# rogeliorjr/DyCON_Paper_Replication

Hardware: AMD Instinct MI355X
Metric: train volumes/sec (96^3 patch) (higher is better)
Workload: dtype bf16

## Files before the change

### dycon_paper_replication_amd/_lib.py

```python
from __future__ import annotations

import ctypes as C
import os

_HERE = os.path.dirname(os.path.abspath(__file__))
LIB_PATH = os.environ.get("DYCON_LIB", os.path.join(_HERE, "libdycon_hip.so"))

F32, BF16 = 0, 1
CONV_1X1, CONV_K3, CONV_K2S2 = 0, 1, 2

P, I, L, F, Z, U64 = C.c_void_p, C.c_int, C.c_longlong, C.c_float, C.c_size_t, C.c_uint64

SIGNATURES = {
    "dycon_version": (I, []),
    "dycon_last_error": (C.c_char_p, []),
    "dycon_bfrag_bytes": (Z, [I, I, I, I]),
    "dycon_pack_bfrag": (I, [P, P, I, I, I, I, I, L, L, L, L, I, P]),
    "dycon_pack_batch": (I, [P, I, I, P]),
    "dycon_pack_tcn": (I, [P, P, I, I, I, I, L, L, L, L, I, P]),
    "dycon_conv_gemm_workspace": (Z, [I, I, I, I, I, I, I, I, I]),
    "dycon_conv_gemm_plan": (I, [I, I, I, I, I, I, I, I, I, I, I, P]),
    "dycon_conv_kernel_name": (C.c_char_p, [I]),
    "dycon_conv_region_name": (C.c_char_p, [P]),
    "dycon_conv_gemm": (I, [P, P, P, P, I, I, I, I, I, I, I, I, I, I, I, P, Z, P]),
    "dycon_conv_gemm_splits": (I, [I, I, I, I, I, I, I, I, I]),
    "dycon_conv_gemm_ex": (I, [P, P, P, P, I, I, I, I, I, I, I, I, I, I, I, P, Z, I, P]),
    "dycon_conv_direct": (I, [P, I, P, P, P, I, I, I, I, I, I, I, I, I, P]),
    "dycon_conv_wgrad_workspace": (Z, [I, I, I, I, I, I, I]),
    "dycon_conv_wgrad_name": (C.c_char_p, [I, I, I, I, I, I, I, I, I]),
    "dycon_conv_wgrad": (I, [P, I, P, I, P, P, I, I, I, I, I, I, I, L, L, L, P, Z, P]),
    "dycon_colsum_workspace": (Z, [L, I]),
    "dycon_colsum": (I, [P, I, P, L, I, P, Z, P]),
    "dycon_norm_workspace": (Z, [I, L, I]),
    "dycon_norm_stats": (I, [P, I, I, L, I, I, F, P, P, P, F, P, Z, P]),
    "dycon_norm_fwd": (I, [P, P, I, I, L, I, I, F, P, P, P, I, P, P, P, P, F, P, Z, P]),
    "dycon_norm_fwd_is_fused": (I, [I, L, I, I]),
    "dycon_norm_fwd_slab": (I, [P, I, P, P, P, I, I, L, I, I, F, P, P, P, I, P, P, P]),
    "dycon_norm_apply": (I, [P, P, I, I, L, I, I, P, P, P, I, P, P, P]),
    "dycon_norm_bwd": (I, [P, I, P, P, I, I, L, I, I, P, P, P, I, P, P, P, P, Z, P]),
    "dycon_norm_bwd_ex": (I, [P, I, P, P, I, I, L, I, I, P, P, P, I, P, P, P, I, P, Z, P]),
    "dycon_norm_sum_dparams": (I, [P, I, I, P, P, P]),
    "dycon_norm_head_workspace": (Z, [I, L]),
    "dycon_norm_head_fwd": (I, [P, I, I, L, I, P, P, P, I, P, P, P, P, P]),
    "dycon_norm_head_bwd": (I, [P, P, P, I, I, L, I, P, P, P, I, P, P, P, P, P, Z, P]),
    "dycon_norm_head_dparams": (I, [P, I, L, P, P, P]),
    "dycon_norm_headc_workspace": (Z, [I, L, I]),
    "dycon_norm_headc_fwd": (I, [P, I, I, L, I, I, P, P, P, I, P, P, P, P, P]),
# ... 106 lines not shown
    "dycon_sample_colsum": (I, [P, I, P, I, L, I, F, I, P]),
    "dycon_sample_bcast": (I, [P, P, P, I, I, L, I, F, P]),
    "dycon_small_gemm": (I, [P, L, L, P, L, L, P, L, I, I, I, I, P]),
    "dycon_copy_segments": (I, [P, P, P, I, P]),
    "dycon_assemble_batch": (I, [P, P, P, I, I, I, I, P, P, I, P]),
    "dycon_sw_gather": (I, [P, I, I, I, P, I, I, I, I, I, I, P, P]),
    "dycon_sw_accumulate_ens": (I, [P, P, P, P, I, I, I, I, I, I, P, P, P, I, I, I, P]),
    "dycon_volume_stats_workspace": (Z, [I, L]),
    "dycon_volume_stats": (I, [P, I, L, P, P, P, Z, P]),
    "dycon_normalize_apply": (I, [P, I, L, P, P, P]),
    "dycon_zoom_workspace": (Z, [I, I, I, I]),
    "dycon_zoom": (I, [P, I, I, I, I, I, I, I, I, I, P, I, F, P, I, P, Z, P]),
    "dycon_kernel_timing": (I, [I]),
    "dycon_kernel_timing_count": (L, []),
    "dycon_kernel_timing_fetch": (I, [L, L, P, P, P]),
    "dycon_kernel_timing_name": (C.c_char_p, [I]),
}


class ConvPlan(C.Structure):
    _fields_ = [("family", I), ("splits", I), ("chunks", I), ("weights", I), ("workspace", Z)]


CONV_NONE, CONV_C1, CONV_P16, CONV_P32, CONV_LDS, CONV_HALO, CONV_TILE, CONV_GEMM = range(8)
CONV_W_FRAG, CONV_W_CHUNK16 = 0, 1


class View(C.Structure):
    _fields_ = [("p", P), ("sn", L), ("sc", L), ("sv", L)]


class DyconLibraryError(RuntimeError):
    pass


_lib = None


def load():
    global _lib
    if _lib is not None:
        return _lib
    if not os.path.exists(LIB_PATH):
        raise DyconLibraryError(
            f"{LIB_PATH} not found: the HIP extension is not built.  Run "
            "`python -c 'import __graft_entry__ as g; g.build()'` from the repo root.  "
            "There is no CPU/PyTorch fallback for the DyCON hot path.")
# ... 95 lines not shown
```

### dycon_paper_replication_amd/csrc/conv.hip

```cpp
#include <stdlib.h>

#include "common.h"

typedef float f32x4 __attribute__((ext_vector_type(4)));
typedef __bf16 bf16x8 __attribute__((ext_vector_type(8)));

template <typename T> struct Frag;
template <> struct Frag<float> { static constexpr int G = 4, KC = 16; };
template <> struct Frag<bf16> { static constexpr int G = 8, KC = 32; };

__device__ __forceinline__ void mma(f32x4& acc, const Vec16<float>& a, const Vec16<float>& b) {
    acc = __builtin_amdgcn_mfma_f32_16x16x4f32(a.v.x, b.v.x, acc, 0, 0, 0);
    acc = __builtin_amdgcn_mfma_f32_16x16x4f32(a.v.y, b.v.y, acc, 0, 0, 0);
    acc = __builtin_amdgcn_mfma_f32_16x16x4f32(a.v.z, b.v.z, acc, 0, 0, 0);
    acc = __builtin_amdgcn_mfma_f32_16x16x4f32(a.v.w, b.v.w, acc, 0, 0, 0);
}
__device__ __forceinline__ void mma(f32x4& acc, const Vec16<bf16>& a, const Vec16<bf16>& b) {
    acc = __builtin_amdgcn_mfma_f32_16x16x32_bf16(__builtin_bit_cast(bf16x8, a.v), __builtin_bit_cast(bf16x8, b.v),
                                                  acc, 0, 0, 0);
}

template <int MODE> __device__ __forceinline__ int n_taps() { return MODE == DYCON_CONV_K3 ? 27 : MODE == DYCON_CONV_K2S2 ? 8 : 1; }

template <int MODE>
__device__ __forceinline__ bool src_voxel(int t, int z, int y, int x, int Di, int Hi, int Wi, int& zi, int& yi, int& xi) {
    if (MODE == DYCON_CONV_K3) {
        const int dz = t / 9, dy = (t / 3) % 3, dx = t % 3;
        zi = z + dz - 1; yi = y + dy - 1; xi = x + dx - 1;
        return (unsigned)zi < (unsigned)Di && (unsigned)yi < (unsigned)Hi && (unsigned)xi < (unsigned)Wi;
    } else if (MODE == DYCON_CONV_K2S2) {
        zi = 2 * z + (t >> 2); yi = 2 * y + ((t >> 1) & 1); xi = 2 * x + (t & 1);
        return true;
    } else {
        zi = z; yi = y; xi = x;
        return true;
    }
}

template <typename T>
__global__ void pack_bfrag_kernel(const float* __restrict__ w, T* __restrict__ out, int Tn, int Cin, int N, int N0,
                                  long long s_t, long long s_c, long long s_n1, long long s_n0, int flip, int NT,
                                  long long total) {
    constexpr int G = Frag<T>::G, KC = Frag<T>::KC;
    for (long long i = (long long)blockIdx.x * blockDim.x + threadIdx.x; i < total; i += (long long)gridDim.x * blockDim.x) {
        const int e = (int)(i % G);
        long long q = i / G;
        const int lane = (int)(q % 64);
        q /= 64;
        const int nt = (int)(q % NT);
        const int kc = (int)(q / NT);
        const int k = kc * KC + G * (lane >> 4) + e;
        const int n = nt * 16 + (lane & 15);
        float v = 0.f;
        if (k < Tn * Cin && n < N) {
            int t = k / Cin;
            const int c = k - t * Cin;
            if (flip) t = Tn - 1 - t;
            v = w[t * s_t + c * s_c + (long long)(n / N0) * s_n1 + (long long)(n % N0) * s_n0];
        }
        stf(out + i, v);
// ... 2548 lines not shown
    if (!(B > 0 && Di > 0 && Hi > 0 && Wi > 0 && Cin > 0 && N > 0 && Cout > 0)) return {"conv_gemm: bad shape", 0};
    if (mode < 0 || mode > 2) return {"conv_gemm: bad mode %d", mode};
    if (!conv_first_layer(dtype, mode, scatter, Di, Hi, Wi, Cin, Cout) && Cin % (dtype == DYCON_BF16 ? 8 : 4) != 0)
        return {"conv_gemm: Cin=%d not a multiple of the fragment width", Cin};
    if (N % 16 != 0) return {"conv_gemm: N=%d not a multiple of 16 (use dycon_conv_direct)", N};
    if (scatter && !(mode == DYCON_CONV_1X1 && N == 8 * Cout)) return {"conv_gemm: scatter needs mode 1x1 and N == 8*Cout", 0};
    if (!scatter && N != Cout) return {"conv_gemm: N must equal Cout without scatter", 0};
    if (mode == DYCON_CONV_K2S2 && (Di % 2 || Hi % 2 || Wi % 2)) return {"conv_gemm: k2s2 needs even dims", 0};
    return {nullptr, 0};
}
struct ConvPlan {
    int family = DYCON_CONV_NONE;
    int variant = 0;
    int ck = 0, ntb = 0;
    bool wide = false;
    int tz = 0, ty = 0, tx = 0, nTiles = 0;
    dim3 grid;
    long long M = 0;
    SplitK sk{1, 0};
    int splits = 1;
    size_t ws_bytes = 0;
    int chunks = 0;
    int weights = DYCON_CONV_W_FRAG;
};
static ConvPlan conv_fwd_plan(int dtype, int mode, int scatter, int accumulate, int B, int Di, int Hi, int Wi, int Cin, int N, int Cout) {
    ConvPlan p;
    if (B <= 0 || Di <= 0 || Hi <= 0 || Wi <= 0 || Cin <= 0 || N <= 0 || Cout <= 0 || mode < 0 || mode > 2) return p;
    int Do, Ho, Wo;
    row_grid(mode, Di, Hi, Wi, Do, Ho, Wo);
    p.M = (long long)B * Do * Ho * Wo;
    if (p.M <= 0) return p;
    const long long DHW = (long long)Di * Hi * Wi;
    const bool bf16_k3 = dtype == DYCON_BF16 && mode == DYCON_CONV_K3 && !scatter;
    const bool first_layer = conv_first_layer(dtype, mode, scatter, Di, Hi, Wi, Cin, Cout);
    if (first_layer || (bf16_k3 && DHW >= CONV_LDS_MIN_VOXELS && (Cin == 16 || Cin == 48 || Cin % 32 == 0) && (Cout == 16 || Cout == 32 || Cout % 64 == 0 || Cout % 48 == 0))) {
        p.tz = cdiv(Di, CL_TZ); p.ty = cdiv(Hi, CL_TY); p.tx = cdiv(Wi, CL_TX);
        p.nTiles = B * p.tz * p.ty * p.tx;
        if (first_layer || (Cin == 16 && Cout == 16)) {
            p.family = first_layer ? DYCON_CONV_C1 : DYCON_CONV_P16;
            p.variant = Cout / 16;
            p.grid = dim3(8 * min(cdiv(p.nTiles, 8), first_layer ? 128 : 32 * P16_WGS));
            p.chunks = (Cout == 16 && !accumulate) ? (int)p.grid.x : 0;
        } else if (Cin == 32 && Cout == 32 && !accumulate && p.nTiles >= 1024) {
            p.family = DYCON_CONV_P32;
            p.grid = dim3(8 * min(cdiv(p.nTiles, 8), 32));
            p.chunks = (int)p.grid.x;
        } else {
// ... 7 lines not shown
        }
        return p;
    }
    if (bf16_k3 && Cin % 32 == 0 && N % CT_BN == 0 && Cin >= 64 && DHW < CONV_LDS_MIN_VOXELS) {
        p.sk = conv_tile_plan(p.M, N, Cin);
        if (Cin == CH_CIN && p.sk.splits <= CH_MAXS) {
            p.family = DYCON_CONV_HALO;
            p.variant = p.sk.splits > 2 ? 2 : 1;
            p.tz = cdiv(Di, CH_T); p.ty = cdiv(Hi, CH_T); p.tx = cdiv(Wi, CH_T);
            p.nTiles = B * p.tz * p.ty * p.tx;
            p.grid = dim3(p.nTiles, N / 64);
            return p;
        }
        p.family = DYCON_CONV_TILE;
        p.variant = (Cin % 64 == 0 && p.sk.kc_per_split % 2 == 0) ? 2 : 1;
        p.grid = dim3(cdiv(p.M, CT_BM), N / CT_BN, p.sk.splits);
    } else {
        p.family = DYCON_CONV_GEMM;
        p.sk = splitk_plan(dtype, mode, scatter, p.M, N, Cin);
        p.grid = dim3(cdiv(p.M, 64), cdiv((N + 15) / 16, NTB), p.sk.splits);
    }
    p.splits = p.sk.splits;
    if (p.splits > 1) p.ws_bytes = (size_t)p.splits * p.M * N * sizeof(float);
    return p;
}

extern "C" int dycon_pack_batch(const dycon_pack_job_t* jobs_dev, int njobs, int blocks_per_job, dycon_stream_t stream) {
    DYCON_REQUIRE(jobs_dev && njobs > 0 && njobs <= 65535 && blocks_per_job > 0, "pack_batch: bad arguments");
    pack_batch_kernel<<<dim3(blocks_per_job, njobs), 256, 0, stream>>>(jobs_dev);
    DYCON_LAUNCH_CHECK();
    return DYCON_OK;
}

template <typename T>
static void launch_splitk_finish(const float* slabs, const ConvPlan& p, int N, const float* bias, void* y, int accumulate, dycon_stream_t stream) {
    long long blocks = (p.M * N / 4 + 255) / 256;
    if (blocks > 2048) blocks = 2048;
    splitk_finish_kernel<T><<<(int)blocks, 256, 0, stream>>>(slabs, p.splits, p.M * N, N, bias, (T*)y, accumulate);
}

template <typename T, int MODE, bool SC>
static void launch_gemm(const ConvPlan& p, const void* x, const void* wf, const float* bias, void* y, int accumulate, int B, int Di, int Hi,
                        int Wi, int Cin, int N, int Cout, float* slabs, int defer_finish, dycon_stream_t stream) {
    int Do, Ho, Wo;
    row_grid(MODE, Di, Hi, Wi, Do, Ho, Wo);
    const int NT = (N + 15) / 16;
    const int Tn = MODE == DYCON_CONV_K3 ? 27 : MODE == DYCON_CONV_K2S2 ? 8 : 1;
    const int nKC = (Tn * Cin + Frag<T>::KC - 1) / Frag<T>::KC;
    conv_gemm_kernel<T, MODE, SC><<<dim3(p.grid.x, p.grid.y, slabs ? p.splits : 1), 256, 0, stream>>>(
        (const T*)x, (const T*)wf, bias, (T*)y, B, Di, Hi, Wi, Cin, Do, Ho, Wo, N, Cout, NT, nKC, accumulate, slabs, p.sk.kc_per_split,
        slabs && defer_finish && N % 8 == 0);
    if (slabs && !defer_finish) launch_splitk_finish<T>(slabs, p, N, bias, y, accumulate, stream);
}

extern "C" int dycon_conv_gemm_plan(int dtype, int mode, int scatter, int accumulate, int B, int Di, int Hi, int Wi, int Cin, int N,
                                    int Cout, dycon_conv_plan_t* out) {
    DYCON_REQUIRE(out, "conv_gemm_plan: null pointer");
    const ConvPlan p = conv_fwd_plan(dtype, mode, scatter, accumulate, B, Di, Hi, Wi, Cin, N, Cout);
    out->family = conv_refusal(dtype, mode, scatter, B, Di, Hi, Wi, Cin, N, Cout).fmt ? DYCON_CONV_NONE : p.family;
    out->splits = p.splits;
    out->chunks = p.chunks;
    out->weights = p.weights;
    out->workspace = p.ws_bytes;
    return DYCON_OK;
}

extern "C" const char* dycon_conv_kernel_name(int family) {
    static const char* const names[] = {"none", "conv_k3_c1", "conv_k3_p16", "conv_k3_p32", "conv_k3_lds", "conv_k3_halo", "conv_k3_tile", "conv_gemm"};
    return family >= 0 && family <= DYCON_CONV_GEMM ? names[family] : "?";
}
extern "C" const char* dycon_conv_region_name(const dycon_conv_plan_t* plan) {
    if (!plan) return "?";
    return plan->family == DYCON_CONV_GEMM && plan->splits > 1 ? "conv_gemm_splitk" : dycon_conv_kernel_name(plan->family);
}

extern "C" size_t dycon_conv_gemm_workspace(int dtype, int mode, int scatter, int B, int Di, int Hi, int Wi, int Cin, int N) {
    return conv_fwd_plan(dtype, mode, scatter, 0, B, Di, Hi, Wi, Cin, N, scatter ? N / 8 : N).ws_bytes;
}
extern "C" int dycon_conv_gemm_splits(int dtype, int mode, int scatter, int B, int Di, int Hi, int Wi, int Cin, int N) {
    return conv_fwd_plan(dtype, mode, scatter, 0, B, Di, Hi, Wi, Cin, N, scatter ? N / 8 : N).splits;
}
extern "C" int dycon_conv_stats_chunks(int dtype, int mode, int B, int Di, int Hi, int Wi, int Cin, int Cout) {
    return conv_fwd_plan(dtype, mode, 0, 0, B, Di, Hi, Wi, Cin, Cout, Cout).chunks;
}

static int conv_fwd_launch(const void* x, const void* wfrag, const float* bias, void* y, int dtype, int mode, int scatter, int accumulate,
                           int B, int Di, int Hi, int Wi, int Cin, int N, int Cout, float* workspace, size_t ws_bytes, int defer_finish,
                           float* stat_part, dycon_stream_t stream) {
    DYCON_REQUIRE(x && wfrag && y, "conv_gemm: null pointer");
    const ConvRefusal no = conv_refusal(dtype, mode, scatter, B, Di, Hi, Wi, Cin, N, Cout);
    DYCON_REQUIRE(!no.fmt, no.fmt, no.arg);
    const ConvPlan p = conv_fwd_plan(dtype, mode, scatter, accumulate, B, Di, Hi, Wi, Cin, N, Cout);
    DYCON_REQUIRE(!defer_finish || (!accumulate && workspace && p.splits > 1 && ws_bytes >= p.ws_bytes),
                  "conv_gemm: defer_finish needs a split-K shape, its workspace and no accumulation");
    const bf16 *xp = (const bf16*)x, *wp = (const bf16*)wfrag;
    bf16* yp = (bf16*)y;
    float* slabs = (p.splits > 1 && workspace && ws_bytes >= p.ws_bytes) ? workspace : nullptr;
    switch (p.family) {
    case DYCON_CONV_C1:
#define DYCON_C1(NTV, STV) conv_k3_c1_kernel<NTV, STV><<<p.grid, 256, 0, stream>>>(xp, wp, bias, yp, B, Di, Hi, Wi, p.tz, p.ty, p.tx, p.nTiles, accumulate, stat_part)
        if (stat_part) DYCON_C1(1, true);
        else if (p.variant == 1) DYCON_C1(1, false);
        else if (p.variant == 2) DYCON_C1(2, false);
        else DYCON_C1(4, false);
#undef DYCON_C1
        break;
    case DYCON_CONV_P16:
#define DYCON_P16(ACCV, STV) conv_k3_p16_kernel<P16_DEPTH, ACCV, STV><<<p.grid, 256, 0, stream>>>(xp, wp, bias, yp, B, Di, Hi, Wi, p.tz, p.ty, p.tx, p.nTiles, stat_part)
        if (accumulate) DYCON_P16(true, false);
        else if (stat_part) DYCON_P16(false, true);
        else DYCON_P16(false, false);
#undef DYCON_P16
        break;
    case DYCON_CONV_P32:
#define DYCON_P32(STV) conv_k3_p32_kernel<8, STV><<<p.grid, 64 * 8, 0, stream>>>(xp, wp, bias, yp, B, Di, Hi, Wi, p.tz, p.ty, p.tx, p.nTiles, stat_part)
        if (stat_part) DYCON_P32(true); else DYCON_P32(false);
#undef DYCON_P32
        break;
    case DYCON_CONV_LDS:
#define DYCON_CL(CKV, NTBV, WMV) \
    conv_k3_lds_kernel<CKV, NTBV, WMV><<<p.grid, 256, 0, stream>>>(xp, wp, bias, yp, B, Di, Hi, Wi, Cin, Cout, Cout / 16, p.tz, p.ty, p.tx, accumulate)
        if (p.ck == 16) {
            if (p.ntb == 1) DYCON_CL(16, 1, 4); else if (p.ntb == 2) DYCON_CL(16, 2, 4); else if (p.ntb == 3) DYCON_CL(16, 3, 4); else DYCON_CL(16, 4, 2);
        } else {
            if (p.ntb == 1) DYCON_CL(32, 1, 4); else if (p.ntb == 2) DYCON_CL(32, 2, 4); else if (p.ntb == 3) DYCON_CL(32, 3, 4);
            else if (p.wide)
                conv_k3_lds_kernel<32, 4, 4, 8><<<p.grid, 512, 0, stream>>>(xp, wp, bias, yp, B, Di, Hi, Wi, Cin, Cout, Cout / 16, p.tz, p.ty, p.tx, accumulate);
            else DYCON_CL(32, 4, 2);
        }
#undef DYCON_CL
        break;
    case DYCON_CONV_HALO:
#define DYCON_CH(NJV) conv_k3_halo_kernel<NJV><<<p.grid, 64 * CH_NW, 0, stream>>>(xp, wp, bias, yp, Di, Hi, Wi, N, N / 16, p.tz, p.ty, p.tx, p.sk.splits, p.sk.kc_per_split, accumulate)
        if (p.variant == 2) DYCON_CH(2); else DYCON_CH(1);
#undef DYCON_CH
        break;
    case DYCON_CONV_TILE: {
        const dim3 grid(p.grid.x, p.grid.y, slabs ? p.splits : 1);
#define DYCON_CT(KV) conv_k3_tile_kernel<KV><<<grid, 256, 0, stream>>>(xp, wp, bias, yp, slabs, B, Di, Hi, Wi, Cin, N, N / 16, 27 * Cin / 32, p.sk.kc_per_split, accumulate, slabs && defer_finish ? 1 : 0)
        if (p.variant == 2) DYCON_CT(2); else DYCON_CT(1);
#undef DYCON_CT
        DYCON_LAUNCH_CHECK();
        if (slabs && !defer_finish) launch_splitk_finish<bf16>(slabs, p, N, bias, y, accumulate, stream);
        break;
    }
    default:
        DYCON_DISPATCH(dtype, {
            if (scatter) launch_gemm<T, DYCON_CONV_1X1, true>(p, x, wfrag, bias, y, accumulate, B, Di, Hi, Wi, Cin, N, Cout, slabs, defer_finish, stream);
            else if (mode == DYCON_CONV_K3) launch_gemm<T, DYCON_CONV_K3, false>(p, x, wfrag, bias, y, accumulate, B, Di, Hi, Wi, Cin, N, Cout, slabs, defer_finish, stream);
            else if (mode == DYCON_CONV_K2S2) launch_gemm<T, DYCON_CONV_K2S2, false>(p, x, wfrag, bias, y, accumulate, B, Di, Hi, Wi, Cin, N, Cout, slabs, defer_finish, stream);
            else launch_gemm<T, DYCON_CONV_1X1, false>(p, x, wfrag, bias, y, accumulate, B, Di, Hi, Wi, Cin, N, Cout, slabs, defer_finish, stream);
        });
    }
    DYCON_LAUNCH_CHECK();
    return DYCON_OK;
}

extern "C" int dycon_conv_gemm_ex(const void* x, const void* wfrag, const float* bias, void* y, int dtype, int mode,
                                  int scatter, int accumulate, int B, int Di, int Hi, int Wi, int Cin, int N, int Cout,
                                  float* workspace, size_t ws_bytes, int defer_finish, dycon_stream_t stream) {
    return conv_fwd_launch(x, wfrag, bias, y, dtype, mode, scatter, accumulate, B, Di, Hi, Wi, Cin, N, Cout, workspace, ws_bytes, defer_finish,
                           nullptr, stream);
}

extern "C" int dycon_conv_gemm(const void* x, const void* wfrag, const float* bias, void* y, int dtype, int mode,
                               int scatter, int accumulate, int B, int Di, int Hi, int Wi, int Cin, int N, int Cout,
                               float* workspace, size_t ws_bytes, dycon_stream_t stream) {
    return conv_fwd_launch(x, wfrag, bias, y, dtype, mode, scatter, accumulate, B, Di, Hi, Wi, Cin, N, Cout, workspace, ws_bytes, 0, nullptr,
                           stream);
}

extern "C" int dycon_conv_gemm_stats(const void* x, const void* wfrag, const float* bias, void* y, int dtype, int B, int Di, int Hi,
                                     int Wi, int Cin, int Cout, float* stat_part, size_t stat_bytes, dycon_stream_t stream) {
    const int chunks = dycon_conv_stats_chunks(dtype, DYCON_CONV_K3, B, Di, Hi, Wi, Cin, Cout);
    DYCON_REQUIRE(chunks > 0, "conv_gemm_stats: shape not served (ask dycon_conv_stats_chunks)");
    DYCON_REQUIRE(stat_part && stat_bytes >= (size_t)B * chunks * Cout * 2 * sizeof(float), "conv_gemm_stats: statistics buffer too small");
    return conv_fwd_launch(x, wfrag, bias, y, dtype, DYCON_CONV_K3, 0, 0, B, Di, Hi, Wi, Cin, Cout, Cout, nullptr, 0, 0, stat_part, stream);
}

template <typename TI, typename TO>
static void launch_direct(const void* x, const float* w, const float* bias, void* y, int mode, int accumulate, int B, int Di,
                          int Hi, int Wi, int Cin, int N, dycon_stream_t stream) {
    int Do, Ho, Wo;
    row_grid(mode, Di, Hi, Wi, Do, Ho, Wo);
    const long long M = (long long)B * Do * Ho * Wo;
    const int grid = cdiv(M, 256);
#define DYCON_DIRECT(MODE) \
    conv_direct_kernel<TI, TO, MODE><<<grid, 256, 0, stream>>>((const TI*)x, w, bias, (TO*)y, B, Di, Hi, Wi, Cin, Do, Ho, Wo, N, accumulate)
    if (mode == DYCON_CONV_K3) DYCON_DIRECT(DYCON_CONV_K3);
    else if (mode == DYCON_CONV_K2S2) DYCON_DIRECT(DYCON_CONV_K2S2);
    else DYCON_DIRECT(DYCON_CONV_1X1);
#undef DYCON_DIRECT
// ... 320 lines not shown
```

### dycon_paper_replication_amd/ops.py

```python
from __future__ import annotations

import collections
import ctypes
import functools
from typing import Optional

import torch

from . import _lib
from ._lib import BF16, CONV_1X1, CONV_K2S2, CONV_K3, F32, call, query

_DT = {torch.float32: F32, torch.bfloat16: BF16}


def dt(t: torch.Tensor) -> int:
    try:
        return _DT[t.dtype]
    except KeyError:
        raise TypeError(f"unsupported dtype {t.dtype}: the HIP path stores fp32 or bf16") from None


_STREAMS = []


# ... 224 lines not shown
    def __init__(self, ws, splits, bias):
        self.ws, self.splits, self.bias = ws, splits, bias


_TAPS = {CONV_K3: 27, CONV_K2S2: 8, CONV_1X1: 1}


def conv_gemm(x, wfrag, bias, mode, N, Cout, scatter=False, out=None, accumulate=False, defer_finish=False):
    B, D, H, W, Cin = x.shape
    plan = conv_plan_for(x, mode, N, Cout, scatter, accumulate)
    if defer_finish:
        assert out is None and not accumulate and not scatter
        if plan.splits <= 1:
            return conv_gemm(x, wfrag, bias, mode, N, Cout), None
    if out is None:
        assert not accumulate
        if scatter:
            shape = (B, 2 * D, 2 * H, 2 * W, Cout)
        elif mode == CONV_K2S2:
            shape = (B, D // 2, H // 2, W // 2, N)
        else:
            shape = (B, D, H, W, N)
        out = torch.empty(shape, dtype=x.dtype, device=x.device)
    nws = plan.workspace
    ws = _ws(nws, x) if nws else None
    args = (_p(x), _p(wfrag), _p(bias), _p(out), dt(x), mode, int(scatter), int(accumulate), B, D, H, W, Cin, N, Cout, _p(ws), nws)
    if PROFILER is None and not defer_finish:
        call("dycon_conv_gemm", *args, _s())
        return out
    rows = out.numel() // Cout if not scatter else x.numel() // Cin
    with _Region(plan.name, (x.numel() + out.numel() * (2 if accumulate else 1)) * _es(x) + _TAPS[mode] * Cin * N * _es(x),
                 2 * rows * _TAPS[mode] * Cin * N):
        call("dycon_conv_gemm_ex", *args, int(defer_finish), _s())
    return (out, DeferredConv(ws, plan.splits, bias)) if defer_finish else out


def conv_stats_chunks(x, Cin, Cout):
    return conv_plan_for(x, CONV_K3, Cout, Cout).chunks


def conv_gemm_stats(x, wfrag, bias, Cout, chunks):
    B, D, H, W, Cin = x.shape
    y = torch.empty((B, D, H, W, Cout), dtype=x.dtype, device=x.device)
    part = torch.empty(B * chunks * Cout * 2, dtype=torch.float32, device=x.device)
    with _Region(conv_plan_for(x, CONV_K3, Cout, Cout).name, (x.numel() + y.numel()) * _es(x) + 27 * Cin * Cout * _es(x),
                 2 * (y.numel() // Cout) * 27 * Cin * Cout):
        call("dycon_conv_gemm_stats", _p(x), _p(wfrag), _p(bias), _p(y), dt(x), B, D, H, W, Cin, Cout, _p(part), part.numel() * 4, _s())
# ... 672 lines not shown
```

### include/dycon_hip.h

```cpp
#ifndef DYCON_HIP_H
#define DYCON_HIP_H

#include <stddef.h>
#include <stdint.h>

#ifdef __cplusplus
extern "C" {
#endif

typedef struct ihipStream_t* dycon_stream_t;

#define DYCON_F32 0
#define DYCON_BF16 1

#define DYCON_OK 0
#define DYCON_ERR_INVALID (-22)
#define DYCON_ERR_LAUNCH (-5)

#define DYCON_CONV_1X1 0
#define DYCON_CONV_K3 1
#define DYCON_CONV_K2S2 2

int dycon_version(void);
const char* dycon_last_error(void);

size_t dycon_bfrag_bytes(int dtype, int T, int Cin, int N);
int dycon_pack_bfrag(const float* w, void* out, int dtype, int T, int Cin, int N, int N0,
                     long long s_t, long long s_c, long long s_n1, long long s_n0, int flip_taps,
                     dycon_stream_t stream);
typedef struct {
    const float* w;
    void* out;
    long long s_t, s_c, s_n1, s_n0, total;
    int kind, T, Cin, N, N0, flip, NT, pad_;
} dycon_pack_job_t;
int dycon_pack_batch(const dycon_pack_job_t* jobs_dev, int njobs, int blocks_per_job, dycon_stream_t stream);
int dycon_pack_tcn(const float* w, float* out, int T, int Cin, int N, int N0, long long s_t,
                   long long s_c, long long s_n1, long long s_n0, int flip_taps, dycon_stream_t stream);

enum {
    DYCON_CONV_NONE = 0, DYCON_CONV_C1, DYCON_CONV_P16, DYCON_CONV_P32, DYCON_CONV_LDS, DYCON_CONV_HALO, DYCON_CONV_TILE,
    DYCON_CONV_GEMM
};
enum { DYCON_CONV_W_FRAG = 0, DYCON_CONV_W_CHUNK16 = 1 };
typedef struct {
    int family, splits, chunks, weights;
    size_t workspace;
} dycon_conv_plan_t;
int dycon_conv_gemm_plan(int dtype, int mode, int scatter, int accumulate, int B, int Di, int Hi, int Wi, int Cin, int N,
                         int Cout, dycon_conv_plan_t* plan);
const char* dycon_conv_kernel_name(int family);
const char* dycon_conv_region_name(const dycon_conv_plan_t* plan);
size_t dycon_conv_gemm_workspace(int dtype, int mode, int scatter, int B, int Di, int Hi, int Wi,
                                 int Cin, int N);
int dycon_conv_gemm(const void* x, const void* wfrag, const float* bias, void* y, int dtype,
                    int mode, int scatter, int accumulate, int B, int Di, int Hi, int Wi, int Cin,
                    int N, int Cout, float* workspace, size_t ws_bytes, dycon_stream_t stream);
int dycon_conv_gemm_splits(int dtype, int mode, int scatter, int B, int Di, int Hi, int Wi, int Cin, int N);
int dycon_conv_gemm_ex(const void* x, const void* wfrag, const float* bias, void* y, int dtype,
                       int mode, int scatter, int accumulate, int B, int Di, int Hi, int Wi, int Cin,
                       int N, int Cout, float* workspace, size_t ws_bytes, int defer_finish,
                       dycon_stream_t stream);
int dycon_conv_direct(const void* x, int x_dtype, const float* w_tcn, const float* bias, void* y,
                      int y_dtype, int mode, int accumulate, int B, int Di, int Hi, int Wi, int Cin,
                      int N, dycon_stream_t stream);

size_t dycon_conv_wgrad_workspace(int mode, int B, int Di, int Hi, int Wi, int Cin, int Cout);
const char* dycon_conv_wgrad_name(int x_dtype, int g_dtype, int mode, int B, int Di, int Hi, int Wi, int Cin, int Cout);
int dycon_conv_wgrad(const void* x, int x_dtype, const void* gy, int g_dtype, float* dw, float* dbias,
                     int mode, int B, int Di, int Hi, int Wi, int Cin, int Cout, long long s_t,
                     long long s_c, long long s_n, float* workspace, size_t ws_bytes,
                     dycon_stream_t stream);

size_t dycon_colsum_workspace(long long rows, int C);
int dycon_colsum(const void* x, int dtype, float* out, long long rows, int C, float* workspace,
                 size_t ws_bytes, dycon_stream_t stream);

size_t dycon_norm_workspace(int Nb, long long V, int C);
int dycon_norm_stats(const void* x, int dtype, int Nb, long long V, int C, int G, float eps,
                     float* stats, float* running_mean, float* running_var, float momentum,
                     float* workspace, size_t ws_bytes, dycon_stream_t stream);
int dycon_norm_fwd(const void* x, void* y, int dtype, int Nb, long long V, int C, int G, float eps,
                   float* stats, const float* gamma, const float* beta, int relu, const void* skip,
                   const float* chan_scale, float* running_mean, float* running_var, float momentum,
                   float* workspace, size_t ws_bytes, dycon_stream_t stream);
// ... 340 lines not shown
```

Before: 925.8.

## Add in-workgroup split-K conv kernels reducing partials through LDS

Adds two new forward conv kernels for small deep layers (k3 with Cin 256 and k2s2 downsampling) where split-K is needed. Each kernel puts all K splits in separate waves of one workgroup and reduces the partial sums in LDS, instead of writing fp32 slabs to global memory and running a separate finish pass. This removes the workspace traffic and the extra launch for those shapes, at the cost of large LDS use per workgroup, lower occupancy and a narrower set of shapes that qualify. A slabs entry point keeps the old global-workspace path available for callers that defer the finish.

```diff
diff --git a/dycon_paper_replication_amd/_lib.py b/dycon_paper_replication_amd/_lib.py
--- a/dycon_paper_replication_amd/_lib.py
+++ b/dycon_paper_replication_amd/_lib.py
@@ -23,6 +23,7 @@
     "dycon_conv_kernel_name": (C.c_char_p, [I]),
     "dycon_conv_region_name": (C.c_char_p, [P]),
     "dycon_conv_gemm": (I, [P, P, P, P, I, I, I, I, I, I, I, I, I, I, I, P, Z, P]),
+    "dycon_conv_gemm_slabs": (I, [P, P, P, P, I, I, I, I, I, I, I, I, I, I, I, P, Z, P]),
     "dycon_conv_gemm_splits": (I, [I, I, I, I, I, I, I, I, I]),
     "dycon_conv_gemm_ex": (I, [P, P, P, P, I, I, I, I, I, I, I, I, I, I, I, P, Z, I, P]),
     "dycon_conv_direct": (I, [P, I, P, P, P, I, I, I, I, I, I, I, I, I, P]),
@@ -175,7 +176,9 @@
     _fields_ = [("family", I), ("splits", I), ("chunks", I), ("weights", I), ("workspace", Z)]
 
 
-CONV_NONE, CONV_C1, CONV_P16, CONV_P32, CONV_LDS, CONV_HALO, CONV_TILE, CONV_GEMM = range(8)
+(CONV_NONE, CONV_C1, CONV_P16, CONV_P32, CONV_LDS, CONV_HALO, CONV_TILE, CONV_GEMM, CONV_K3_WGSPLIT,
+ CONV_K2S2_WGSPLIT) = range(10)
+CONV_WGSPLIT = (CONV_K3_WGSPLIT, CONV_K2S2_WGSPLIT)
 CONV_W_FRAG, CONV_W_CHUNK16 = 0, 1
 
 
diff --git a/dycon_paper_replication_amd/csrc/conv.hip b/dycon_paper_replication_amd/csrc/conv.hip
--- a/dycon_paper_replication_amd/csrc/conv.hip
+++ b/dycon_paper_replication_amd/csrc/conv.hip
@@ -1,41 +1,6 @@
 #include <stdlib.h>
 
-#include "common.h"
-
-typedef float f32x4 __attribute__((ext_vector_type(4)));
-typedef __bf16 bf16x8 __attribute__((ext_vector_type(8)));
-
-template <typename T> struct Frag;
-template <> struct Frag<float> { static constexpr int G = 4, KC = 16; };
-template <> struct Frag<bf16> { static constexpr int G = 8, KC = 32; };
-
-__device__ __forceinline__ void mma(f32x4& acc, const Vec16<float>& a, const Vec16<float>& b) {
-    acc = __builtin_amdgcn_mfma_f32_16x16x4f32(a.v.x, b.v.x, acc, 0, 0, 0);
-    acc = __builtin_amdgcn_mfma_f32_16x16x4f32(a.v.y, b.v.y, acc, 0, 0, 0);
-    acc = __builtin_amdgcn_mfma_f32_16x16x4f32(a.v.z, b.v.z, acc, 0, 0, 0);
-    acc = __builtin_amdgcn_mfma_f32_16x16x4f32(a.v.w, b.v.w, acc, 0, 0, 0);
-}
-__device__ __forceinline__ void mma(f32x4& acc, const Vec16<bf16>& a, const Vec16<bf16>& b) {
-    acc = __builtin_amdgcn_mfma_f32_16x16x32_bf16(__builtin_bit_cast(bf16x8, a.v), __builtin_bit_cast(bf16x8, b.v),
-                                                  acc, 0, 0, 0);
-}
-
-template <int MODE> __device__ __forceinline__ int n_taps() { return MODE == DYCON_CONV_K3 ? 27 : MODE == DYCON_CONV_K2S2 ? 8 : 1; }
-
-template <int MODE>
-__device__ __forceinline__ bool src_voxel(int t, int z, int y, int x, int Di, int Hi, int Wi, int& zi, int& yi, int& xi) {
-    if (MODE == DYCON_CONV_K3) {
-        const int dz = t / 9, dy = (t / 3) % 3, dx = t % 3;
-        zi = z + dz - 1; yi = y + dy - 1; xi = x + dx - 1;
-        return (unsigned)zi < (unsigned)Di && (unsigned)yi < (unsigned)Hi && (unsigned)xi < (unsigned)Wi;
-    } else if (MODE == DYCON_CONV_K2S2) {
-        zi = 2 * z + (t >> 2); yi = 2 * y + ((t >> 1) & 1); xi = 2 * x + (t & 1);
-        return true;
-    } else {
-        zi = z; yi = y; xi = x;
-        return true;
-    }
-}
+#include "conv_mma.h"
 
 template <typename T>
 __global__ void pack_bfrag_kernel(const float* __restrict__ w, T* __restrict__ out, int Tn, int Cin, int N, int N0,
@@ -2630,7 +2595,29 @@
     size_t ws_bytes = 0;
     int chunks = 0;
     int weights = DYCON_CONV_W_FRAG;
+    int slab_family = DYCON_CONV_NONE;
+    int mt = 0;
 };
+constexpr int CONV_CUS = 256;
+static void conv_wgsplit_plan(ConvPlan& p, int dtype, int mode, int scatter, int B, int Di, int Hi, int Wi, int Cin, int N) {
+    if (dtype != DYCON_BF16 || scatter || p.sk.splits < 2 || N % WS_COLS != 0) return;
+    if (p.family == DYCON_CONV_TILE && Cin == WS_K3_CIN && p.sk.splits <= WS_K3_MAXS && p.sk.kc_per_split % 2 == 0) {
+        const int tz = cdiv(Di, WS_T), ty = cdiv(Hi, WS_T), tx = cdiv(Wi, WS_T);
+        const long long wgs = (long long)B * tz * ty * tx * (N / WS_COLS);
+        if (wgs < CONV_CUS / 2 || wgs > CONV_CUS) return;
+        p.slab_family = p.family;
+        p.family = DYCON_CONV_K3_WGSPLIT;
+        p.tz = tz; p.ty = ty; p.tx = tx;
+        p.nTiles = B * tz * ty * tx;
+    } else if (p.family == DYCON_CONV_GEMM && mode == DYCON_CONV_K2S2 && Cin % 32 == 0 && p.sk.splits <= WS_MAX_WAVES) {
+        const int mt = p.sk.splits <= 4 ? 4 : p.sk.splits <= 8 ? 2 : 1;
+        const long long wgs = (long long)cdiv(p.M, 16 * mt) * (N / WS_COLS);
+        if (wgs < CONV_CUS / 2 || wgs * mt * p.sk.splits > CONV_CUS * WS_MAX_WAVES) return;
+        p.slab_family = p.family;
+        p.family = DYCON_CONV_K2S2_WGSPLIT;
+        p.mt = mt;
+    }
+}
 static ConvPlan conv_fwd_plan(int dtype, int mode, int scatter, int accumulate, int B, int Di, int Hi, int Wi, int Cin, int N, int Cout) {
     ConvPlan p;
     if (B <= 0 || Di <= 0 || Hi <= 0 || Wi <= 0 || Cin <= 0 || N <= 0 || Cout <= 0 || mode < 0 || mode > 2) return p;
@@ -2684,6 +2671,7 @@
     }
     p.splits = p.sk.splits;
     if (p.splits > 1) p.ws_bytes = (size_t)p.splits * p.M * N * sizeof(float);
+    conv_wgsplit_plan(p, dtype, mode, scatter, B, Di, Hi, Wi, Cin, N);
     return p;
 }
 
@@ -2728,8 +2716,9 @@
 }
 
 extern "C" const char* dycon_conv_kernel_name(int family) {
-    static const char* const names[] = {"none", "conv_k3_c1", "conv_k3_p16", "conv_k3_p32", "conv_k3_lds", "conv_k3_halo", "conv_k3_tile", "conv_gemm"};
-    return family >= 0 && family <= DYCON_CONV_GEMM ? names[family] : "?";
+    static const char* const names[] = {"none", "conv_k3_c1", "conv_k3_p16", "conv_k3_p32", "conv_k3_lds", "conv_k3_halo", "conv_k3_tile", "conv_gemm",
+                                        "conv_k3_wgsplit", "conv_k2s2_wgsplit"};
+    return family >= 0 && family <= DYCON_CONV_K2S2_WGSPLIT ? names[family] : "?";
 }
 extern "C" const char* dycon_conv_region_name(const dycon_conv_plan_t* plan) {
     if (!plan) return "?";
@@ -2748,7 +2737,7 @@
 
 static int conv_fwd_launch(const void* x, const void* wfrag, const float* bias, void* y, int dtype, int mode, int scatter, int accumulate,
                            int B, int Di, int Hi, int Wi, int Cin, int N, int Cout, float* workspace, size_t ws_bytes, int defer_finish,
-                           float* stat_part, dycon_stream_t stream) {
+                           float* stat_part, dycon_stream_t stream, int as_slabs = 0) {
     DYCON_REQUIRE(x && wfrag && y, "conv_gemm: null pointer");
     const ConvRefusal no = conv_refusal(dtype, mode, scatter, B, Di, Hi, Wi, Cin, N, Cout);
     DYCON_REQUIRE(!no.fmt, no.fmt, no.arg);
@@ -2758,7 +2747,9 @@
     const bf16 *xp = (const bf16*)x, *wp = (const bf16*)wfrag;
     bf16* yp = (bf16*)y;
     float* slabs = (p.splits > 1 && workspace && ws_bytes >= p.ws_bytes) ? workspace : nullptr;
-    switch (p.family) {
+    DYCON_REQUIRE(!as_slabs || p.splits <= 1 || slabs, "conv_gemm_slabs: a split-K shape needs its workspace");
+    const bool wgsplit = p.slab_family != DYCON_CONV_NONE && !defer_finish && !as_slabs;
+    switch (wgsplit || p.slab_family == DYCON_CONV_NONE ? p.family : p.slab_family) {
     case DYCON_CONV_C1:
 #define DYCON_C1(NTV, STV) conv_k3_c1_kernel<NTV, STV><<<p.grid, 256, 0, stream>>>(xp, wp, bias, yp, B, Di, Hi, Wi, p.tz, p.ty, p.tx, p.nTiles, accumulate, stat_part)
         if (stat_part) DYCON_C1(1, true);
@@ -2797,6 +2788,12 @@
         if (p.variant == 2) DYCON_CH(2); else DYCON_CH(1);
 #undef DYCON_CH
         break;
+    case DYCON_CONV_K3_WGSPLIT:
+        conv_k3_wgsplit_launch(xp, wp, bias, yp, B, Di, Hi, Wi, N, p.tz, p.ty, p.tx, p.sk.splits, p.sk.kc_per_split, accumulate, stream);
+        break;
+    case DYCON_CONV_K2S2_WGSPLIT:
+        conv_k2s2_wgsplit_launch(xp, wp, bias, yp, B, Di, Hi, Wi, Cin, N, p.mt, p.sk.splits, p.sk.kc_per_split, accumulate, stream);
+        break;
     case DYCON_CONV_TILE: {
         const dim3 grid(p.grid.x, p.grid.y, slabs ? p.splits : 1);
 #define DYCON_CT(KV) conv_k3_tile_kernel<KV><<<grid, 256, 0, stream>>>(xp, wp, bias, yp, slabs, B, Di, Hi, Wi, Cin, N, N / 16, 27 * Cin / 32, p.sk.kc_per_split, accumulate, slabs && defer_finish ? 1 : 0)
@@ -2830,6 +2827,13 @@
                                float* workspace, size_t ws_bytes, dycon_stream_t stream) {
     return conv_fwd_launch(x, wfrag, bias, y, dtype, mode, scatter, accumulate, B, Di, Hi, Wi, Cin, N, Cout, workspace, ws_bytes, 0, nullptr,
                            stream);
+}
+
+extern "C" int dycon_conv_gemm_slabs(const void* x, const void* wfrag, const float* bias, void* y, int dtype, int mode,
+                                     int scatter, int accumulate, int B, int Di, int Hi, int Wi, int Cin, int N, int Cout,
+                                     float* workspace, size_t ws_bytes, dycon_stream_t stream) {
+    return conv_fwd_launch(x, wfrag, bias, y, dtype, mode, scatter, accumulate, B, Di, Hi, Wi, Cin, N, Cout, workspace, ws_bytes, 0, nullptr,
+                           stream, 1);
 }
 
 extern "C" int dycon_conv_gemm_stats(const void* x, const void* wfrag, const float* bias, void* y, int dtype, int B, int Di, int Hi,
diff --git a/dycon_paper_replication_amd/csrc/conv_mma.h b/dycon_paper_replication_amd/csrc/conv_mma.h
--- /dev/null
+++ b/dycon_paper_replication_amd/csrc/conv_mma.h
@@ -0,0 +1,47 @@
+#pragma once
+#include "common.h"
+
+typedef float f32x4 __attribute__((ext_vector_type(4)));
+typedef __bf16 bf16x8 __attribute__((ext_vector_type(8)));
+
+template <typename T> struct Frag;
+template <> struct Frag<float> { static constexpr int G = 4, KC = 16; };
+template <> struct Frag<bf16> { static constexpr int G = 8, KC = 32; };
+
+__device__ __forceinline__ void mma(f32x4& acc, const Vec16<float>& a, const Vec16<float>& b) {
+    acc = __builtin_amdgcn_mfma_f32_16x16x4f32(a.v.x, b.v.x, acc, 0, 0, 0);
+    acc = __builtin_amdgcn_mfma_f32_16x16x4f32(a.v.y, b.v.y, acc, 0, 0, 0);
+    acc = __builtin_amdgcn_mfma_f32_16x16x4f32(a.v.z, b.v.z, acc, 0, 0, 0);
+    acc = __builtin_amdgcn_mfma_f32_16x16x4f32(a.v.w, b.v.w, acc, 0, 0, 0);
+}
+__device__ __forceinline__ void mma(f32x4& acc, const Vec16<bf16>& a, const Vec16<bf16>& b) {
+    acc = __builtin_amdgcn_mfma_f32_16x16x32_bf16(__builtin_bit_cast(bf16x8, a.v), __builtin_bit_cast(bf16x8, b.v),
+                                                  acc, 0, 0, 0);
+}
+
+template <int MODE> __device__ __forceinline__ int n_taps() { return MODE == DYCON_CONV_K3 ? 27 : MODE == DYCON_CONV_K2S2 ? 8 : 1; }
+
+template <int MODE>
+__device__ __forceinline__ bool src_voxel(int t, int z, int y, int x, int Di, int Hi, int Wi, int& zi, int& yi, int& xi) {
+    if (MODE == DYCON_CONV_K3) {
+        const int dz = t / 9, dy = (t / 3) % 3, dx = t % 3;
+        zi = z + dz - 1; yi = y + dy - 1; xi = x + dx - 1;
+        return (unsigned)zi < (unsigned)Di && (unsigned)yi < (unsigned)Hi && (unsigned)xi < (unsigned)Wi;
+    } else if (MODE == DYCON_CONV_K2S2) {
+        zi = 2 * z + (t >> 2); yi = 2 * y + ((t >> 1) & 1); xi = 2 * x + (t & 1);
+        return true;
+    } else {
+        zi = z; yi = y; xi = x;
+        return true;
+    }
+}
+
+constexpr int WS_T = 4;
+constexpr int WS_K3_CIN = 256;
+constexpr int WS_K3_MAXS = 18;
+constexpr int WS_COLS = 32;
+constexpr int WS_MAX_WAVES = 16;
+void conv_k3_wgsplit_launch(const bf16* x, const bf16* wf, const float* bias, bf16* y, int B, int D, int H, int W, int N, int tz, int ty,
+                            int tx, int S, int kc_per_split, int accumulate, hipStream_t stream);
+void conv_k2s2_wgsplit_launch(const bf16* x, const bf16* wf, const float* bias, bf16* y, int B, int Di, int Hi, int Wi, int Cin, int N,
+                              int MT, int S, int kc_per_split, int accumulate, hipStream_t stream);
diff --git a/dycon_paper_replication_amd/csrc/conv_small.hip b/dycon_paper_replication_amd/csrc/conv_small.hip
--- /dev/null
+++ b/dycon_paper_replication_amd/csrc/conv_small.hip
@@ -0,0 +1,247 @@
+#include "conv_mma.h"
+
+constexpr int WS_H = WS_T + 2, WS_NH = WS_H * WS_H * WS_H;
+constexpr int WS_ROW = WS_K3_CIN * 2;
+constexpr int WS_NW = 8;
+constexpr int WS_RPW = (WS_K3_MAXS + WS_NW - 1) / WS_NW;
+constexpr int WS_HALO_BYTES = WS_NH * WS_ROW;
+constexpr int WS_RED_BYTES = WS_K3_MAXS * 8 * 1024;
+constexpr int WS_MAIN_BYTES = WS_HALO_BYTES > WS_RED_BYTES ? WS_HALO_BYTES : WS_RED_BYTES;
+constexpr int WS_OP = WS_COLS + 8;
+
+__global__ __launch_bounds__(64 * WS_NW, 1)
+void conv_k3_wgsplit_kernel(const bf16* __restrict__ X, const bf16* __restrict__ Wf, const float* __restrict__ bias, bf16* __restrict__ Y,
+                            int D, int H, int W, int N, int NT, int tz, int ty, int tx, int S, int kc_per_split, int accumulate) {
+    constexpr int KS = 27 * WS_K3_CIN / 32;
+    __shared__ __attribute__((aligned(16))) unsigned char lds[WS_MAIN_BYTES + 64 * WS_OP * 2];
+    unsigned short* ot = reinterpret_cast<unsigned short*>(lds + WS_MAIN_BYTES);
+    const int tid = threadIdx.x, lane = tid & 63, wave = tid >> 6;
+    const int r = lane & 15, kg = lane >> 4, ry = r >> 2, rx = r & 3;
+    int q = blockIdx.x;
+    const int bx = q % tx; q /= tx;
+    const int by = q % ty; q /= ty;
+    const int bz = q % tz;
+    const int b = q / tz;
+    const int z0 = bz * WS_T, y0 = by * WS_T, x0 = bx * WS_T;
+    const int nt0 = blockIdx.y * 2;
+    const bf16* xb = X + (long long)b * D * H * W * WS_K3_CIN;
+
+    {
+        constexpr int PIECES = WS_NH * 32, PER = 7;
+        static_assert(2 * PER * 64 * WS_NW >= PIECES, "halo staging covers every piece");
+#pragma unroll
+        for (int pass = 0; pass < 2; ++pass) {
+            uint4 v[PER];
+#pragma unroll
+            for (int i = 0; i < PER; ++i) {
+                const int p = tid + (pass * PER + i) * 64 * WS_NW, hv = p >> 5, sl = p & 31;
+                const int hz = hv / 36, hy = (hv / 6) % 6, hx = hv % 6;
+                const int zi = z0 + hz - 1, yi = y0 + hy - 1, xi = x0 + hx - 1;
+                v[i] = make_uint4(0, 0, 0, 0);
+                if (p < PIECES && (unsigned)zi < (unsigned)D && (unsigned)yi < (unsigned)H && (unsigned)xi < (unsigned)W)
+                    v[i] = *reinterpret_cast<const uint4*>(xb + (((long long)zi * H + yi) * W + xi) * WS_K3_CIN + sl * 8);
+            }
+#pragma unroll
+            for (int i = 0; i < PER; ++i) {
+                const int p = tid + (pass * PER + i) * 64 * WS_NW, hv = p >> 5, sl = p & 31;
+                const int hy = (hv / 6) % 6, hx = hv % 6;
+                if (p < PIECES) *reinterpret_cast<uint4*>(lds + hv * WS_ROW + ((sl ^ (4 * (hy & 3) + (hx & 3))) * 16)) = v[i];
+            }
+        }
+    }
+
+    auto load_b = [&](int kc, uint4 (&bf)[2]) {
+        const uint4* p = reinterpret_cast<const uint4*>(Wf + ((long long)kc * NT + nt0) * 512) + lane;
+        bf[0] = p[0];
+        bf[1] = p[64];
+    };
+    f32x4 acc[WS_RPW][4][2];
+#pragma unroll
+    for (int ri = 0; ri < WS_RPW; ++ri)
+#pragma unroll
+        for (int m = 0; m < 4; ++m)
+#pragma unroll
+            for (int j = 0; j < 2; ++j) acc[ri][m][j] = f32x4{0.f, 0.f, 0.f, 0.f};
+    auto compute = [&](int kc, const uint4 (&bf)[2], f32x4 (&ac)[4][2]) {
+        const int t = kc >> 3, kq = kc & 7;
+        const int dz = t / 9, dy = (t / 3) % 3, dx = t % 3;
+        const int hy = ry + dy, hx = rx + dx;
+        const int slot = (4 * kq + kg) ^ (4 * (hy & 3) + (hx & 3));
+        const unsigned char* ap = lds + ((dz * WS_H + hy) * WS_H + hx) * WS_ROW + slot * 16;
+        bf16x8 a[4];
+#pragma unroll
+        for (int m = 0; m < 4; ++m) a[m] = __builtin_bit_cast(bf16x8, *reinterpret_cast<const uint4*>(ap + m * WS_H * WS_H * WS_ROW));
+#pragma unroll
+        for (int m = 0; m < 4; ++m)
+#pragma unroll
+            for (int j = 0; j < 2; ++j) ac[m][j] = __builtin_amdgcn_mfma_f32_16x16x32_bf16(a[m], __builtin_bit_cast(bf16x8, bf[j]), ac[m][j], 0, 0, 0);
+    };
+
+    __syncthreads();
+#pragma unroll
+    for (int ri = 0; ri < WS_RPW; ++ri) {
+        const int zs = wave + WS_NW * ri;
+        const int k0 = zs * kc_per_split, k1 = min(KS, k0 + kc_per_split);
+        if (zs < S && k0 < k1) {
+            uint4 s0[2][2], s1[2][2];
+            auto load_pair = [&](int kc, uint4 (&s)[2][2]) {
+                const int kp = min(kc, k1 - 2);
+                load_b(kp, s[0]);
+                load_b(kp + 1, s[1]);
+            };
+            load_pair(k0, s0);
+            load_pair(k0 + 2, s1);
+            int kc = k0;
+            for (; kc + 4 <= k1; kc += 4) {
+                compute(kc, s0[0], acc[ri]);
+                compute(kc + 1, s0[1], acc[ri]);
+                load_pair(kc + 4, s0);
+                compute(kc + 2, s1[0], acc[ri]);
+                compute(kc + 3, s1[1], acc[ri]);
+                load_pair(kc + 6, s1);
+            }
+            if (kc < k1) {
+                compute(kc, s0[0], acc[ri]);
+                compute(kc + 1, s0[1], acc[ri]);
+            }
+        }
+    }
+    __syncthreads();
+
+    float* red = reinterpret_cast<float*>(lds);
+#pragma unroll
+    for (int ri = 0; ri < WS_RPW; ++ri) {
+        const int zs = wave + WS_NW * ri;
+        if (zs < S) {
+#pragma unroll
+            for (int m = 0; m < 4; ++m)
+#pragma unroll
+                for (int j = 0; j < 2; ++j) *reinterpret_cast<f32x4*>(red + zs * 2048 + ((m * 2 + j) * 64 + lane) * 4) = acc[ri][m][j];
+        }
+    }
+    __syncthreads();
+    {
+        const int T = tid >> 6, rm = T >> 1, rj = T & 1;
+        const int col = rj * 16 + r;
+        const int n = nt0 * 16 + col;
+        const float bv = bias ? bias[n] : 0.f;
+        f32x4 o = f32x4{bv, bv, bv, bv};
+        for (int z = 0; z < S; ++z) o += *reinterpret_cast<const f32x4*>(red + z * 2048 + tid * 4);
+#pragma unroll
+        for (int i = 0; i < 4; ++i) {
+            const int row = rm * 16 + kg * 4 + i;
+            float v = o[i];
+            if (accumulate) {
+                const int zo = z0 + rm, yo = y0 + kg, xo = x0 + i;
+                if (zo < D && yo < H && xo < W) v += ldf(Y + ((((long long)b * D + zo) * H + yo) * W + xo) * N + n);
+            }
+            ot[row * WS_OP + col] = f32_to_bf16_bits(v);
+        }
+    }
+    __syncthreads();
+    if (tid < 256) {
+        const int row = tid >> 2, pc = tid & 3;
+        const int zo = z0 + (row >> 4), yo = y0 + ((row >> 2) & 3), xo = x0 + (row & 3);
+        if (zo < D && yo < H && xo < W)
+            *reinterpret_cast<uint4*>(Y + ((((long long)b * D + zo) * H + yo) * W + xo) * N + nt0 * 16 + pc * 8) =
+                *reinterpret_cast<const uint4*>(ot + row * WS_OP + pc * 8);
+    }
+}
+
+void conv_k3_wgsplit_launch(const bf16* x, const bf16* wf, const float* bias, bf16* y, int B, int D, int H, int W, int N, int tz, int ty,
+                            int tx, int S, int kc_per_split, int accumulate, hipStream_t stream) {
+    conv_k3_wgsplit_kernel<<<dim3(B * tz * ty * tx, N / WS_COLS), 64 * WS_NW, 0, stream>>>(x, wf, bias, y, D, H, W, N, N / 16, tz, ty, tx, S,
+                                                                                          kc_per_split, accumulate);
+}
+
+constexpr int WS_UB = 8;
+
+__global__ __launch_bounds__(64 * WS_MAX_WAVES)
+void conv_k2s2_wgsplit_kernel(const bf16* __restrict__ X, const bf16* __restrict__ Wf, const float* __restrict__ bias, bf16* __restrict__ Y,
+                              int Di, int Hi, int Wi, int Cin, long long M, int N, int NT, int nKC, int MT, int S, int kc_per_split,
+                              int accumulate) {
+    extern __shared__ __attribute__((aligned(16))) unsigned char wlds[];
+    const int lane = threadIdx.x & 63, wave = threadIdx.x >> 6;
+    const int r = lane & 15, kg = lane >> 4;
+    const int zs = wave / MT, mt = wave - zs * MT;
+    const int Do = Di >> 1, Ho = Hi >> 1, Wo = Wi >> 1;
+    const long long m0 = ((long long)blockIdx.x * MT + mt) * 16;
+    const long long m = m0 + r;
+    const bool mvalid = m < M;
+    int xo, yo, zo, bo;
+    {
+        long long q = mvalid ? m : 0;
+        xo = (int)(q % Wo); q /= Wo;
+        yo = (int)(q % Ho); q /= Ho;
+        zo = (int)(q % Do);
+        bo = (int)(q / Do);
+    }
+    const int nt0 = blockIdx.y * 2;
+    const int kc0 = zs * kc_per_split, kc1 = min(nKC, kc0 + kc_per_split);
+    int t = (kc0 * 32) / Cin, c = kc0 * 32 - t * Cin;
+    const bf16* xa = X + ((((long long)bo * Di + 2 * zo) * Hi + 2 * yo) * Wi + 2 * xo) * Cin + 8 * kg;
+    const uint4* wf = reinterpret_cast<const uint4*>(Wf) + ((long long)kc0 * NT + nt0) * 64 + lane;
+    f32x4 acc[2] = {f32x4{0.f, 0.f, 0.f, 0.f}, f32x4{0.f, 0.f, 0.f, 0.f}};
+    for (int kcb = kc0; kcb < kc1; kcb += WS_UB) {
+        uint4 a[WS_UB], bq[WS_UB][2];
+#pragma unroll
+        for (int u = 0; u < WS_UB; ++u) {
+            a[u] = make_uint4(0, 0, 0, 0);
+            if (kcb + u < kc1) {
+                if (mvalid) a[u] = *reinterpret_cast<const uint4*>(xa + ((long long)((t >> 2) * Hi + ((t >> 1) & 1)) * Wi + (t & 1)) * Cin + c);
+                bq[u][0] = wf[0];
+                bq[u][1] = wf[64];
+                wf += (long long)NT * 64;
+                c += 32;
+                if (c == Cin) { c = 0; ++t; }
+            }
+        }
+#pragma unroll
+        for (int u = 0; u < WS_UB; ++u) {
+            if (kcb + u < kc1) {
+#pragma unroll
+                for (int j = 0; j < 2; ++j)
+                    acc[j] = __builtin_amdgcn_mfma_f32_16x16x32_bf16(__builtin_bit_cast(bf16x8, a[u]), __builtin_bit_cast(bf16x8, bq[u][j]), acc[j], 0, 0, 0);
+            }
+        }
+    }
+
+    float* red = reinterpret_cast<float*>(wlds);
+    unsigned short* ot = reinterpret_cast<unsigned short*>(wlds + (S - 1) * MT * 2048) + mt * 16 * WS_OP;
+    if (zs > 0) {
+#pragma unroll
+        for (int j = 0; j < 2; ++j) *reinterpret_cast<f32x4*>(red + ((((zs - 1) * MT + mt) * 2 + j) * 64 + lane) * 4) = acc[j];
+    }
+    __syncthreads();
+    if (zs == 0) {
+#pragma unroll
+        for (int j = 0; j < 2; ++j) {
+            const int n = (nt0 + j) * 16 + r;
+            const float bv = bias ? bias[n] : 0.f;
+            f32x4 o = f32x4{bv, bv, bv, bv};
+            o += acc[j];
+            for (int z = 1; z < S; ++z) o += *reinterpret_cast<const f32x4*>(red + ((((z - 1) * MT + mt) * 2 + j) * 64 + lane) * 4);
+#pragma unroll
+            for (int i = 0; i < 4; ++i) {
+                const int row = kg * 4 + i;
+                float v = o[i];
+                if (accumulate && m0 + row < M) v += ldf(Y + (m0 + row) * N + n);
+                ot[row * WS_OP + j * 16 + r] = f32_to_bf16_bits(v);
+            }
+        }
+    }
+    __syncthreads();
+    if (zs == 0) {
+        const int row = lane >> 2, pc = lane & 3;
+        if (m0 + row < M)
+            *reinterpret_cast<uint4*>(Y + (m0 + row) * N + nt0 * 16 + pc * 8) = *reinterpret_cast<const uint4*>(ot + row * WS_OP + pc * 8);
+    }
+}
+
+void conv_k2s2_wgsplit_launch(const bf16* x, const bf16* wf, const float* bias, bf16* y, int B, int Di, int Hi, int Wi, int Cin, int N,
+                              int MT, int S, int kc_per_split, int accumulate, hipStream_t stream) {
+    const long long M = (long long)B * (Di / 2) * (Hi / 2) * (Wi / 2);
+    const size_t lds = (size_t)(S - 1) * MT * 2048 + (size_t)MT * 16 * WS_OP * 2;
+    conv_k2s2_wgsplit_kernel<<<dim3(cdiv(M, 16 * MT), N / WS_COLS), 64 * MT * S, lds, stream>>>(x, wf, bias, y, Di, Hi, Wi, Cin, M, N, N / 16,
+                                                                                               8 * Cin / 32, MT, S, kc_per_split, accumulate);
+}
diff --git a/dycon_paper_replication_amd/ops.py b/dycon_paper_replication_amd/ops.py
--- a/dycon_paper_replication_amd/ops.py
+++ b/dycon_paper_replication_amd/ops.py
@@ -270,7 +270,7 @@
         else:
             shape = (B, D, H, W, N)
         out = torch.empty(shape, dtype=x.dtype, device=x.device)
-    nws = plan.workspace
+    nws = plan.workspace if (defer_finish or plan.family not in _lib.CONV_WGSPLIT) else 0
     ws = _ws(nws, x) if nws else None
     args = (_p(x), _p(wfrag), _p(bias), _p(out), dt(x), mode, int(scatter), int(accumulate), B, D, H, W, Cin, N, Cout, _p(ws), nws)
     if PROFILER is None and not defer_finish:
diff --git a/include/dycon_hip.h b/include/dycon_hip.h
--- a/include/dycon_hip.h
+++ b/include/dycon_hip.h
@@ -40,7 +40,7 @@
 
 enum {
     DYCON_CONV_NONE = 0, DYCON_CONV_C1, DYCON_CONV_P16, DYCON_CONV_P32, DYCON_CONV_LDS, DYCON_CONV_HALO, DYCON_CONV_TILE,
-    DYCON_CONV_GEMM
+    DYCON_CONV_GEMM, DYCON_CONV_K3_WGSPLIT, DYCON_CONV_K2S2_WGSPLIT
 };
 enum { DYCON_CONV_W_FRAG = 0, DYCON_CONV_W_CHUNK16 = 1 };
 typedef struct {
@@ -61,6 +61,9 @@
                        int mode, int scatter, int accumulate, int B, int Di, int Hi, int Wi, int Cin,
                        int N, int Cout, float* workspace, size_t ws_bytes, int defer_finish,
                        dycon_stream_t stream);
+int dycon_conv_gemm_slabs(const void* x, const void* wfrag, const float* bias, void* y, int dtype,
+                          int mode, int scatter, int accumulate, int B, int Di, int Hi, int Wi, int Cin,
+                          int N, int Cout, float* workspace, size_t ws_bytes, dycon_stream_t stream);
 int dycon_conv_direct(const void* x, int x_dtype, const float* w_tcn, const float* bias, void* y,
                       int y_dtype, int mode, int accumulate, int B, int Di, int Hi, int Wi, int Cin,
                       int N, dycon_stream_t stream);
```

Result: no change. 931.6, median of 6 (+0.6%).
